# OPPO-Mente-Lab/X2I

Hardware: AMD Instinct MI355X
Metric: images/sec, FLUX-schnell 1024x1024 4-step (projector + denoise loop), whole job (higher is better)
Workload: dtype bf16; 1 GPU; BASELINE configs[1]: qwen3b conditioning (C=37,H=2048,S_txt=512) -> projector -> shuttle-3/FLUX-schnell DiT 1024x1024, 4 steps; batch_per_gpu=4, global_batch=4, parallelism=batch-sharded x1, graph=True

## Files before the change

x2i_amd/csrc/gemm256p.hip:

```cpp
#include <type_traits>
#include "gemm_device.h"
#include "gemm256p_epi.h"
#include "gemm256w_loop.inc"
#include "gemm256f8_loop.inc"

namespace x2i_gemm {
namespace {

__device__ __forceinline__ void epilogue_fx_slice(const GemmP& p, int z, int m_wave, int n_wave, int lane, char* stage, int slab0, int P, int j,
                                                  int tid) {
  typedef unsigned int u32x4 __attribute__((ext_vector_type(4)));
  typedef unsigned int u32x2 __attribute__((ext_vector_type(2)));
  const int mlane = lane & 15, ng = lane >> 4;
  const int srow = lane >> 3, sch = lane & 7;
  const float* b2 = p.bias2 ? p.bias2 + (long long)z * p.bias2_bs : nullptr;
#ifdef X2I_ABLATION
  if (p.act2 >= 80) b2 = nullptr;
#endif
  const float* gz = p.gate ? p.gate + (long long)z * p.gate_bs : nullptr;
  __amdgpu_buffer_rsrc_t r_rsrc = __builtin_amdgcn_make_buffer_rsrc((void*)(p.res + (long long)z * p.r_bs), 0, (uint32_t)(((long long)(p.M - 1) * p.ldr + p.N) * 2), 0x00020000);
  const uint32_t c_bytes = (uint32_t)(((long long)(p.M - 1) * p.ldc + p.N) * 2);
  __amdgpu_buffer_rsrc_t c_rsrc = __builtin_amdgcn_make_buffer_rsrc((void*)((bf16_t*)p.C + (long long)z * p.c_bs), 0, c_bytes, 0x00020000);
  const float* sbase = p.sk_slabs + (long long)slab0 * (SK_SLAB_BYTES / 4) + tid * 4;
  for (int q = j; q < 8; q += P) {
    const int h = q >> 2, c = q & 3;
    float bv[4][4], gv[4][4];
#pragma unroll
    for (int jj = 0; jj < 4; ++jj) {
      const int n = n_wave + h * 64 + jj * 16 + ng * 4;
#pragma unroll
      for (int r = 0; r < 4; ++r) bv[jj][r] = 0.f, gv[jj][r] = 1.f;
      if (n + 3 < p.N) {
        if (p.bias) {
          const uint2 bb = *(const uint2*)(p.bias + n);
          bv[jj][0] = __uint_as_float(bb.x << 16); bv[jj][1] = __uint_as_float(bb.x & 0xffff0000u);
          bv[jj][2] = __uint_as_float(bb.y << 16); bv[jj][3] = __uint_as_float(bb.y & 0xffff0000u);
        }
        if (gz) {
          const f32x4_t g4 = *(const f32x4_t*)(gz + n);
          gv[jj][0] = g4[0]; gv[jj][1] = g4[1]; gv[jj][2] = g4[2]; gv[jj][3] = g4[3];
        }
        if (b2) {
          const f32x4_t t4 = *(const f32x4_t*)(b2 + n);
          bv[jj][0] += t4[0]; bv[jj][1] += t4[1]; bv[jj][2] += t4[2]; bv[jj][3] += t4[3];
        }
      }
    }
    u32x2 rres[2][4];
    const uint32_t rsoff = (uint32_t)(((long long)c * 32 * p.ldr + h * 64) * 2);
#pragma unroll
    for (int i = 0; i < 2; ++i)
#pragma unroll
      for (int jj = 0; jj < 4; ++jj)
        rres[i][jj] = __builtin_amdgcn_raw_buffer_load_b64(r_rsrc, (uint32_t)(((long long)(m_wave + i * 16 + mlane) * p.ldr + n_wave + ng * 4) * 2) + jj * 32, rsoff, 0);
    f32x4_t sum[2][4];
    for (int u = 0; u < P; ++u) {
      const float* su = sbase + (long long)u * 8 * (SK_SLAB_BYTES / 4);
      f32x4_t v[2][4];
#pragma unroll
      for (int i = 0; i < 2; ++i)
#pragma unroll
        for (int jj = 0; jj < 4; ++jj) v[i][jj] = *(const f32x4_t*)(su + ((2 * c + i) * 8 + 4 * h + jj) * 1024);
#pragma unroll
      for (int i = 0; i < 2; ++i)
#pragma unroll
        for (int jj = 0; jj < 4; ++jj) sum[i][jj] = u ? sum[i][jj] + v[i][jj] : v[i][jj];
    }
#pragma unroll
    for (int i = 0; i < 2; ++i) {
      const int row = i * 16 + mlane;
#pragma unroll
      for (int jj = 0; jj < 4; ++jj) {
        float v[4];
#pragma unroll
        for (int r = 0; r < 4; ++r) v[r] = sum[i][jj][r] + bv[jj][r];
        const u32x2 r2 = rres[i][jj];
        v[0] = fmaf(gv[jj][0], v[0], __uint_as_float(r2[0] << 16));
        v[1] = fmaf(gv[jj][1], v[1], __uint_as_float(r2[0] & 0xffff0000u));
        v[2] = fmaf(gv[jj][2], v[2], __uint_as_float(r2[1] << 16));
        v[3] = fmaf(gv[jj][3], v[3], __uint_as_float(r2[1] & 0xffff0000u));
        char* slot = stage + row * 128 + ((((jj << 1) | (ng >> 1)) ^ ((row >> 1) & 7)) << 4) + ((ng & 1) << 3);
        *(uint2*)slot = make_uint2(pack_bf16x2(v[0], v[1]), pack_bf16x2(v[2], v[3]));
      }
    }
    asm volatile("s_waitcnt lgkmcnt(0)" ::: "memory");
    u32x4 d[4];
#pragma unroll
    for (int it = 0; it < 4; ++it) d[it] = *(const u32x4*)(stage + it * 1024 + lane * 16);
    const uint32_t soff = (uint32_t)((long long)c * 32 * p.ldc * 2);
#pragma unroll
    for (int it = 0; it < 4; ++it) {
      const int row = it * 8 + srow;
      const int n = n_wave + h * 64 + ((sch ^ ((row >> 1) & 7)) << 3);
      const uint32_t vo = (n + 7 < p.N) ? (uint32_t)(((long long)(m_wave + row) * p.ldc + n) * 2) : 0x80000000u;
      __builtin_amdgcn_raw_buffer_store_b128(d[it], c_rsrc, vo, soff, 0);
    }
    asm volatile("s_waitcnt lgkmcnt(0)" ::: "memory");
  }
}

template <bool F8 = false>
__device__ __forceinline__ void epilogue_qkv_chunked(const GemmP& p, f32x4_t (&acc)[2][4][2][4], int z, int m_wave, int n_wave, int lane,
                                                     char* stage, const Deq<F8>& dq) {
  asm volatile("" : "+v"(lane));
  const int mlane = lane & 15, ng = lane >> 4;
  const int Dm = p.q_H * 128;
  const int sec = n_wave / Dm;
  const int head = (n_wave - sec * Dm) >> 7;
  uint2 bvp[8];
  static_for<8>([&](auto jc) {
    constexpr int j = decltype(jc)::value;
    const int n = n_wave + j * 16 + ng * 4;
    bvp[j] = (p.bias && n + 3 < p.N) ? *(const uint2*)(p.bias + n) : make_uint2(0u, 0u);
  });
  auto bias_of = [&](int j, int r) {
    const uint32_t u = (r & 2) ? bvp[j].y : bvp[j].x;
    return __uint_as_float((r & 1) ? (u & 0xffff0000u) : (u << 16));
  };
  const TokMap tmap = tok_map(p, z, m_wave);
  auto token = [&](int m, int& b, int& st) { tok_of(tmap, m - m_wave, b, st); };
#ifdef X2I_QKV_ABL
  constexpr int qabl = X2I_QKV_ABL;
#else
  constexpr int qabl = 0;
#endif
  if constexpr (qabl == 92) {
    asm volatile("" ::X2I_GEMM256P_OPS_ACC_IN(acc));
    return;
  }
  if (sec < 2) {
    const int c = lane & 15, rsub = lane >> 4;
    float w[8];
    {
      const bf16x8_t wv = *(const bf16x8_t*)((sec ? p.q_nk : p.q_nq) + c * 8);
#pragma unroll
      for (int j = 0; j < 8; ++j) w[j] = bf16_to_f32((bf16_t)wv[j]) * (sec ? 1.f : p.q_qs);
    }
    typedef unsigned int u32x4 __attribute__((ext_vector_type(4)));
    __amdgpu_buffer_rsrc_t q_rsrc = __builtin_amdgcn_make_buffer_rsrc((void*)(sec ? p.q_K : p.q_Q), 0, 0x7ffffff0u, 0x00020000);
    __amdgpu_buffer_rsrc_t cos_rsrc = __builtin_amdgcn_make_buffer_rsrc((void*)p.q_cos, 0, 0x7ffffff0u, 0x00020000);
    __amdgpu_buffer_rsrc_t sin_rsrc = __builtin_amdgcn_make_buffer_rsrc((void*)p.q_sin, 0, 0x7ffffff0u, 0x00020000);
    auto qk_body = [&](auto pairs_c) {
    constexpr bool pairs = decltype(pairs_c)::value;
    f32x4_t cs[pairs ? 2 : 1][2][4];
    uint32_t qoff[pairs ? 2 : 1][2];
    auto load_cs = [&](int half, auto set_c) {
      constexpr int set = decltype(set_c)::value;
#pragma unroll
      for (int ps = 0; ps < 2; ++ps) {
        const int dm = half * 8 + ps * 4 + rsub;
        const bool valid = m_wave + dm < p.M;
        int b, st;
        tok_of(tmap, valid ? dm : 0, b, st);
        const uint32_t co = (uint32_t)(st * 128 + c * 8) * 4u;
        if constexpr (qabl == 86) {
          cs[set][ps][0] = cs[set][ps][1] = (f32x4_t){1.f, 1.f, 1.f, 1.f};
          cs[set][ps][2] = cs[set][ps][3] = (f32x4_t){0.f, 0.f, 0.f, 0.f};
        } else if constexpr (pairs) {
          cs[set][ps][0] = __builtin_bit_cast(f32x4_t, __builtin_amdgcn_raw_buffer_load_b128(cos_rsrc, co, 0, 0));
          cs[set][ps][1] = __builtin_bit_cast(f32x4_t, __builtin_amdgcn_raw_buffer_load_b128(cos_rsrc, co + 16, 0, 0));
        } else {
          cs[set][ps][0] = __builtin_bit_cast(f32x4_t, __builtin_amdgcn_raw_buffer_load_b128(cos_rsrc, co, 0, 0));
          cs[set][ps][1] = __builtin_bit_cast(f32x4_t, __builtin_amdgcn_raw_buffer_load_b128(cos_rsrc, co + 16, 0, 0));
          cs[set][ps][2] = __builtin_bit_cast(f32x4_t, __builtin_amdgcn_raw_buffer_load_b128(sin_rsrc, co, 0, 0));
          cs[set][ps][3] = __builtin_bit_cast(f32x4_t, __builtin_amdgcn_raw_buffer_load_b128(sin_rsrc, co + 16, 0, 0));
        }
        qoff[set][ps] = valid ? (uint32_t)(((b * p.q_H + head) * p.q_Spad + st) * 128 + c * 8) * 2u : 0x80000000u;
      }
    };
    auto park = [&](auto qc) {
      constexpr int q16 = decltype(qc)::value;
      constexpr int c2 = q16 >> 1, rr = q16 & 1;
      char* buf = stage + (q16 & 1) * 4096;
      static_for<2>([&](auto hc) {
        constexpr int h = decltype(hc)::value;
        static_for<4>([&](auto jc) {
          constexpr int j = decltype(jc)::value;
          float a[4];
#pragma unroll
          for (int r = 0; r < 4; ++r) {
            float t;
            asm volatile("v_accvgpr_read_b32 %0, %1" : "=v"(t) : "a"(acc[h][c2][rr][j][r]));
            if constexpr (F8) a[r] = fmaf(t * dq.sw[h * 4 + j][r], dq.sr[c2][rr], bias_of(h * 4 + j, r));
            else a[r] = t + bias_of(h * 4 + j, r);
          }
          *(uint2*)(buf + mlane * 256 + (((h * 8 + j * 2 + (ng >> 1)) ^ mlane) << 4) + ((ng & 1) << 3)) =
              make_uint2(pack_bf16x2(a[0], a[1]), pack_bf16x2(a[2], a[3]));
        });
      });
    };
    asm volatile("" ::: "memory");
    load_cs(0, std::integral_constant<int, 0>{});
    if constexpr (pairs) load_cs(1, std::integral_constant<int, 1>{});
    park(std::integral_constant<int, 0>{});
    static_for<8>([&](auto qc) {
      constexpr int q16 = decltype(qc)::value;
      char* buf = stage + (q16 & 1) * 4096;
      if constexpr (qabl == 90) {
        if constexpr (q16 + 1 < 8) park(std::integral_constant<int, q16 + 1>{});
        return;
      } else {
      __builtin_amdgcn_sched_barrier(0);
      asm volatile("s_waitcnt lgkmcnt(0)" ::: "memory");
      bf16x8_t xv[4];
#pragma unroll
      for (int k = 0; k < 4; ++k) {
        const int row = k * 4 + rsub;
        xv[k] = *(const bf16x8_t*)(buf + row * 256 + ((c ^ row) << 4));
      }
      __builtin_amdgcn_sched_barrier(0);
      static_for<2>([&](auto hfc) {
        constexpr int hf = decltype(hfc)::value;
        constexpr int half = 2 * q16 + hf;
        constexpr int set = pairs ? (half & 1) : 0;
        u32x4 outv[2];
        uint32_t so[2];
#pragma unroll
        for (int ps = 0; ps < 2; ++ps) {
          float x[8];
#pragma unroll
          for (int j = 0; j < 8; ++j) x[j] = bf16_to_f32((bf16_t)xv[hf * 2 + ps][j]);
          float ss = sumsq8(x);
          if constexpr (qabl != 87) {
#pragma unroll
          for (int o = 8; o > 0; o >>= 1) ss += __shfl_xor(ss, o, 64);
          }
          const float r = rms_rsqrt128(ss, p.q_eps);
          const f32x4_t t0 = cs[set][ps][0], t1 = cs[set][ps][1];
          float csv[8], snv[8];
          if constexpr (pairs) {
            csv[0] = csv[1] = t0[0]; snv[0] = snv[1] = t0[1]; csv[2] = csv[3] = t0[2]; snv[2] = snv[3] = t0[3];
            csv[4] = csv[5] = t1[0]; snv[4] = snv[5] = t1[1]; csv[6] = csv[7] = t1[2]; snv[6] = snv[7] = t1[3];
          } else {
            const f32x4_t t2 = cs[0][ps][2], t3 = cs[0][ps][3];
#pragma unroll
            for (int j = 0; j < 4; ++j) csv[j] = t0[j], csv[4 + j] = t1[j], snv[j] = t2[j], snv[4 + j] = t3[j];
          }
          float o8[8];
          norm_rope8(x, r, w, csv, snv, o8);
#pragma unroll
          for (int j = 0; j < 4; ++j) outv[ps][j] = pack_bf16x2(o8[2 * j], o8[2 * j + 1]);
          so[ps] = qoff[set][ps];
        }
        __builtin_amdgcn_sched_barrier(0);
        if constexpr (pairs) {
          if constexpr (half + 2 < 16) load_cs(half + 2, std::integral_constant<int, set>{});
        } else {
          if constexpr (half + 1 < 16) load_cs(half + 1, std::integral_constant<int, 0>{});
        }
        __builtin_amdgcn_sched_barrier(0);
        if constexpr (qabl != 88) {
#pragma unroll
        for (int ps = 0; ps < 2; ++ps) __builtin_amdgcn_raw_buffer_store_b128(outv[ps], q_rsrc, so[ps], 0, 0);
        } else {
          asm volatile("" ::"v"(outv[0]), "v"(outv[1]));
        }
      });
      if constexpr (q16 + 1 < 8) park(std::integral_constant<int, q16 + 1>{});
      }
    });
    };
    if (p.q_sin == nullptr) qk_body(std::true_type{});
    else qk_body(std::false_type{});
  } else {
    const int ch_lo = lane & 7, dp_lo = lane >> 3;
    const bool aligned = ((p.q_tok_off | p.q_rpb | p.q_row0 | p.M | p.q_Spad) & 7) == 0;
    auto fsw = [](int row) { return ((row >> 3) ^ (row >> 1)) & 7; };
    static_for<4>([&](auto qc) {
      constexpr int q = decltype(qc)::value;
      constexpr int h = q >> 1, cp = q & 1;
      __builtin_amdgcn_sched_barrier(0);
      static_for<2>([&](auto cc) {
        constexpr int c2 = 2 * cp + decltype(cc)::value;
        static_for<2>([&](auto rc) {
          constexpr int rr = decltype(rc)::value;
          const int row = decltype(cc)::value * 32 + rr * 16 + mlane;
          static_for<4>([&](auto jc) {
            constexpr int j = decltype(jc)::value;
            float a[4];
#pragma unroll
            for (int r = 0; r < 4; ++r) {
              float t;
              asm volatile("v_accvgpr_read_b32 %0, %1" : "=v"(t) : "a"(acc[h][c2][rr][j][r]));
              if constexpr (F8) a[r] = fmaf(t * dq.sw[h * 4 + j][r], dq.sr[c2][rr], bias_of(h * 4 + j, r));
              else a[r] = t + bias_of(h * 4 + j, r);
            }
            *(uint2*)(stage + row * 128 + (((j * 2 + (ng >> 1)) ^ fsw(row)) << 4) + ((ng & 1) << 3)) =
                make_uint2(pack_bf16x2(a[0], a[1]), pack_bf16x2(a[2], a[3]));
          });
        });
      });
      asm volatile("s_waitcnt lgkmcnt(0)" ::: "memory");
      if constexpr (qabl == 91) return;
#pragma unroll
      for (int it = 0; it < 4; ++it) {
        const int dp = it * 8 + dp_lo;
        uint32_t v[8];
#pragma unroll
        for (int k = 0; k < 8; ++k) {
          const int row = ch_lo * 8 + k;
          v[k] = *(const uint32_t*)(stage + row * 128 + (((dp >> 2) ^ fsw(row)) << 4) + ((dp & 3) << 2));
        }
        const int m = m_wave + cp * 64 + ch_lo * 8;
        if constexpr (qabl == 89) {
          asm volatile("" ::"v"(v[0]), "v"(v[1]), "v"(v[2]), "v"(v[3]), "v"(v[4]), "v"(v[5]), "v"(v[6]), "v"(v[7]));
        } else if (m < p.M) {
          const int d = h * 64 + dp * 2;
          int b, st;
          token(m, b, st);
          bf16_t* row0 = p.q_VT + (((long long)b * p.q_H + head) * 128 + d) * p.q_Spad;
          if (aligned) {
            union { bf16x8_t v8; uint32_t uu[4]; uint2 h2[2]; } lo, hi;
#pragma unroll
            for (int k = 0; k < 4; ++k) {
              lo.uu[k] = (v[2 * k] & 0xffffu) | (v[2 * k + 1] << 16);
              hi.uu[k] = (v[2 * k] >> 16) | (v[2 * k + 1] & 0xffff0000u);
            }
            if (p.q_vperm) {
              const int ps = x2i_vt_pos(st, 1);
              *(uint2*)(row0 + ps) = lo.h2[0]; *(uint2*)(row0 + ps + 8) = lo.h2[1];
              *(uint2*)(row0 + p.q_Spad + ps) = hi.h2[0]; *(uint2*)(row0 + p.q_Spad + ps + 8) = hi.h2[1];
            } else {
              *(bf16x8_t*)(row0 + st) = lo.v8;
              *(bf16x8_t*)(row0 + p.q_Spad + st) = hi.v8;
            }
          } else {
#pragma unroll
            for (int k = 0; k < 8; ++k) {
              if (m + k < p.M) {
                int bk, sk;
                token(m + k, bk, sk);
                bf16_t* rk = p.q_VT + (((long long)bk * p.q_H + head) * 128 + d) * p.q_Spad + x2i_vt_pos(sk, p.q_vperm);
                rk[0] = (bf16_t)(v[k] & 0xffffu);
                rk[p.q_Spad] = (bf16_t)(v[k] >> 16);
              }
            }
          }
        }
      }
      asm volatile("s_waitcnt lgkmcnt(0)" ::: "memory");
    });
  }
}

struct Unit {
  int vb, k0, len, slab;
  int kind = 0, tag = 0;
};

template <bool PAIR> using GemmArg = std::conditional_t<PAIR, GemmP2, GemmP>;
__device__ __forceinline__ const GemmP& prob(const GemmP& a, int) { return a; }
__device__ __forceinline__ const GemmP& first(const GemmP& a) { return a; }
__device__ __forceinline__ const GemmP& first(const GemmP2& a) { return a.p[0]; }
__device__ __forceinline__ const GemmP& second(const GemmP& a) { return a; }
__device__ __forceinline__ const GemmP& second(const GemmP2& a) { return a.p[1]; }
__device__ __forceinline__ GemmP prob(const GemmP2& a, int sel) {
  const GemmP &x = a.p[0], &y = a.p[1];
  GemmP q;
#define X2I_F(f) q.f = sel ? y.f : x.f;
  X2I_F(A) X2I_F(a_bs) X2I_F(lda) X2I_F(W) X2I_F(ldw) X2I_F(w_bs) X2I_F(bias) X2I_F(C) X2I_F(c_bs) X2I_F(ldc) X2I_F(C2) X2I_F(act2)
  X2I_F(gate) X2I_F(gate_bs) X2I_F(res) X2I_F(r_bs) X2I_F(ldr) X2I_F(bias2) X2I_F(bias2_bs) X2I_F(M) X2I_F(N) X2I_F(K) X2I_F(act)
  X2I_F(out_f32) X2I_F(tilesM) X2I_F(tilesN) X2I_F(cH) X2I_F(cW) X2I_F(cCin) X2I_F(cOW) X2I_F(cKW) X2I_F(cStride) X2I_F(cPad) X2I_F(cUp) X2I_F(cPadW) X2I_F(cRowPitch) X2I_F(cKorder) X2I_F(cMom) X2I_F(cMomBlocks)
  X2I_F(q_on) X2I_F(q_H) X2I_F(q_Spad) X2I_F(q_tok_off) X2I_F(q_rpb) X2I_F(q_row0) X2I_F(q_vperm) X2I_F(gm) X2I_F(q_eps) X2I_F(q_qs) X2I_F(q_nq) X2I_F(q_nk)
  X2I_F(q_cos) X2I_F(q_sin) X2I_F(q_Q) X2I_F(q_K) X2I_F(q_VT) X2I_F(f_sa) X2I_F(f_sa_bs) X2I_F(f_sw) X2I_F(f_alpha) X2I_F(f_oinv) X2I_F(f_out8)
  X2I_F(nbatch) X2I_F(sk_on) X2I_F(sk_slabs) X2I_F(sk_flags) X2I_F(fx_v0)
#undef X2I_F
  return q;
}

template <int ACT, bool RES, bool HASC2, bool QKV = false, bool PAIR = false, bool F8 = false, bool OUT8 = false, bool FX = false>
__global__ __launch_bounds__(256) void gemm256p_kernel(GemmArg<PAIR> pp) {
  constexpr int ES = F8 ? 1 : 2;
  constexpr int KT = F8 ? 128 : BK;
  extern __shared__ __attribute__((aligned(16))) char smem[];
  const GemmP& p = first(pp);
  const int tid = threadIdx.x;
  const int lane = tid & 63;
  const int wave = __builtin_amdgcn_readfirstlane(tid >> 6);
  const int wm = wave >> 1, wn = wave & 1;
  const int TT0 = p.tilesM * p.tilesN * p.nbatch;
  int TT = TT0;
  if constexpr (PAIR) TT += second(pp).tilesM * second(pp).tilesN * second(pp).nbatch;
  const int G = gridDim.x, w = blockIdx.x;
  const int nk = p.K / KT;

  auto tile_of = [&](int vb, int& sel, int& z, int& m0, int& n0) {
    sel = PAIR ? min(max(vb - TT0 + 1, 0), 1) : 0;
    const GemmP& q = prob(pp, sel);
    const int T = q.tilesM * q.tilesN;
    const int v = vb - sel * TT0;
    z = v / T;
    int bid = v - z * T;
    const int qq = T >> 3, r = T & 7, xcd = bid & 7, idx = bid >> 3;
    bid = (xcd < r ? xcd * (qq + 1) : r * (qq + 1) + (xcd - r) * qq) + idx;
    const int GM = q.gm;
    const int per_group = GM * q.tilesN;
    const int group = bid / per_group;
    const int first_m = group * GM;
    const int gsize = min(q.tilesM - first_m, GM);
    m0 = (first_m + (bid % per_group) % gsize) * BM2;
    n0 = ((bid % per_group) / gsize) * BN2;
  };
  const int khl = lane >> 5, r8 = (lane >> 2) & 7, cphys = lane & 3;
  const int kby = khl * 64 + ((cphys ^ (3 * (wave & 1))) << 4);
  auto offsets = [&](int sel, int z, int m0, int n0, uint32_t (&va)[8], uint32_t (&vw)[8]) {
    const GemmP& q = prob(pp, sel);
#ifdef X2I_ABLATION
    if (p.act2 == 75) m0 = 0, n0 = 0;
    if (p.act2 == 76) m0 &= 1023, n0 &= 2047;
#endif
    const long long zoff = (long long)z * q.a_bs;
#pragma unroll
    for (int jj = 0; jj < 8; ++jj) {
      const int row = (jj * 4 + wave) * 8 + r8;
      va[jj] = (m0 + row < q.M) ? (uint32_t)((zoff + (long long)(m0 + row) * q.lda) * ES + kby) : 0x80000000u;
      vw[jj] = (n0 + row < q.N) ? (uint32_t)(((long long)(n0 + row) * q.ldw) * ES + kby) : 0x80000000u;
    }
  };
  auto uni = [](auto v) { return (decltype(v))__builtin_amdgcn_readfirstlane((int)v); };
  auto mk_rsrc = [&](const void* ptr, uint32_t bytes) {
    const unsigned long long a = (unsigned long long)(uintptr_t)ptr;
    const unsigned long long au = ((unsigned long long)(unsigned)uni((int)(a >> 32)) << 32) | (unsigned)uni((int)(a & 0xffffffffu));
    return __builtin_amdgcn_make_buffer_rsrc((void*)(uintptr_t)au, 0, (uint32_t)uni((int)bytes), 0x00020000);
  };
  auto a_rsrc_of = [&](int sel) {
    const GemmP& q = prob(pp, sel);
    return mk_rsrc(q.A, (uint32_t)(((long long)(q.nbatch - 1) * q.a_bs + (long long)(q.M - 1) * q.lda + q.K) * ES));
  };
  auto w_rsrc_of = [&](int sel) {
    const GemmP& q = prob(pp, sel);
    return mk_rsrc(q.W, (uint32_t)(((long long)(q.N - 1) * q.ldw + q.K) * ES));
  };
  int fx_sel = 0, fx_Tp = 0, fx_nbz = 0, fx_kind = 0, fx_cnt = 0, fx_t0 = 0, fx_tstep = 1, fx_k0 = 0, fx_len = 0, fx_npre = 0, fx_modeB = 0, fx_slab_base = 0, fx_part = 0;
  const int fx_x = w & 7;
  if constexpr (FX) {
    const int wi = w >> 3, Gx = G >> 3;
    const int v0 = p.fx_v0;
    fx_sel = PAIR ? min(max(wi - v0 + 1, 0), 1) : 0;
    const GemmP& q = prob(pp, fx_sel);
    const int li = wi - fx_sel * v0, v = fx_sel ? Gx - v0 : v0;
    fx_Tp = q.tilesM * q.tilesN;
    fx_nbz = q.nbatch;
    fx_slab_base = fx_sel * (first(pp).tilesM * first(pp).tilesN);
    const int Tx = fx_Tp >> 3;
    if (v < 2 * Tx) {
      fx_modeB = 1;
      const int nt = v - Tx;
      const int tw = nt > 0 ? (Tx + nt - 1) / nt : 0;
      const int c = nt > 0 ? min(max(nk * tw / (tw + 1), 3), nk - 3) : nk;
      if (li < Tx) {
        fx_kind = 2; fx_cnt = 1; fx_t0 = li; fx_k0 = 0; fx_len = c; fx_npre = nt > 0 ? 1 : 0;
      } else {
        const int j = li - Tx;
        fx_kind = 1; fx_t0 = j; fx_tstep = nt; fx_cnt = (Tx - j + nt - 1) / nt; fx_k0 = c; fx_len = nk - c;
      }
    } else {
      const int base = v / Tx, extra = v - base * Tx;
      const int cutw = extra * (base + 1);
      const int t = li < cutw ? li / (base + 1) : extra + (li - cutw) / base;
      const int P = t < extra ? base + 1 : base;
      const int j = li < cutw ? li - t * (base + 1) : (li - cutw) - (t - extra) * base;
      const int k_lo = (int)((long long)nk * j / P), k_hi = (int)((long long)nk * (j + 1) / P);
      fx_cnt = 1; fx_t0 = t; fx_k0 = k_lo; fx_len = k_hi - k_lo;
      fx_kind = P > 1 ? 3 : 2;
      fx_npre = P - 1;
      fx_part = j;
    }
  }
  int S = TT / G;
  auto hasXlen = [](const Unit& u) { return u.len > 0; };
  Unit segH = {0, 0, 0, -1}, segX = {0, 0, 0, -1};
  int posX = 0;
  if (p.sk_on) {
    const int r = TT - S * G;
    const long long R = (long long)r * nk;
    const int Gp = (int)min((long long)G, R / 6);
    if (w < Gp) {
      auto snap = [&](long long b) {
        const int m = (int)(b % nk);
        return (m != 0 && m < 3) ? b - m : (m > nk - 3 ? b + (nk - m) : b);
      };
      const long long lo = snap(R * w / Gp), hi = snap(R * (w + 1) / Gp);
      if (hi > lo) {
        const int e0 = (int)(lo / nk), e1 = (int)((hi - 1) / nk);
        const int k0 = (int)(lo - (long long)e0 * nk);
        const Unit first = {S * G + e0, k0, (e1 > e0 ? nk : (int)(hi - (long long)e0 * nk)) - k0, e0};
        if (k0 == 0) segH = first; else segX = first;
        if (e1 > e0) segH = Unit{S * G + e1, 0, (int)(hi - (long long)e1 * nk), e1};
        if (segH.len == nk) segH.slab = -1;
        posX = hasXlen(segX) ? min(S, (int)((long long)S * segX.k0 / max(1, nk - segX.len))) : 0;
      }
    }
  } else if (w < TT - S * G) {
    S += 1;
  }
  const int hasH = segH.len > 0, hasX = segX.len > 0;
  const int n_units = FX ? fx_cnt * fx_nbz : S + hasH + hasX;
  auto unit = [&](int i) -> Unit {
    if constexpr (FX) {
      if (i >= n_units) return Unit{-1, 0, 0, -1};
      const int zi = i / fx_cnt, uu = i - zi * fx_cnt;
      const int tile = (fx_t0 + uu * fx_tstep) * 8 + fx_x;
      Unit u;
      u.vb = fx_sel * TT0 + zi * fx_Tp + tile;
      u.k0 = fx_k0;
      u.len = fx_len;
      u.slab = fx_modeB ? fx_slab_base + tile : (fx_kind == 1 ? w : (fx_kind == 3 ? w - 8 * fx_part : w - 8 * fx_npre));
      u.kind = fx_kind;
      u.tag = zi + 1;
      return Unit{uni(u.vb), uni(u.k0), uni(u.len), uni(u.slab), uni(u.kind), uni(u.tag)};
    }
    Unit u{w + (i - hasH) * G, 0, nk, -1};
    if (i >= n_units) u = Unit{-1, 0, 0, -1};
    else if (hasH && i == 0) u = segH;
    else if (hasX) {
      const int j = i - hasH;
      if (j == posX) u = segX;
      else if (j > posX) u.vb -= G;
    }
    return Unit{uni(u.vb), uni(u.k0), uni(u.len), uni(u.slab)};
  };


  const int frow = lane & 15;
  const uint32_t frag = (frow >> 3) * 1024 + (frow & 7) * 64 + (((lane >> 4) ^ (3 * ((frow >> 3) & 1))) << 4);
  uint32_t la = (uint32_t)(uintptr_t)smem + wm * 8 * 2048 + frag;
  uint32_t lw = (uint32_t)(uintptr_t)smem + 32768 + wn * 8 * 2048 + frag;
  uint32_t dma = __builtin_amdgcn_readfirstlane((uint32_t)(uintptr_t)smem + wave * 1024);
  char* stage = smem + P_STAGE_OFF + wave * P_STAGE_WAVE;
  const uint32_t slab_vo = (uint32_t)tid * 16;

  auto slab_rsrc = [&](int slab) {
    const unsigned long long a = (unsigned long long)(uintptr_t)p.sk_slabs + (unsigned long long)slab * SK_SLAB_BYTES;
    const unsigned long long au = ((unsigned long long)(unsigned)uni((int)(a >> 32)) << 32) | (unsigned)uni((int)(a & 0xffffffffu));
    return __builtin_amdgcn_make_buffer_rsrc((void*)(uintptr_t)au, 0, (uint32_t)SK_SLAB_BYTES, 0x00020000);
  };
  if (n_units == 0) return;
#ifdef X2I_ABLATION
  if (p.act2 >= 81 && p.act2 <= 85) {
    int n = (w & 7) * 10;
    if (p.act2 == 82) n = (((w * 167) & 255) * 80) >> 8;
    if (p.act2 == 83) n = (w & 7) * 5;
    if (p.act2 == 85) n = (w & 7) * 20;
    if (p.act2 == 84) {
      for (int i = 0; i < (w & 7) * 5; ++i) __builtin_amdgcn_s_sleep(13);
      n = 0;
    }
    for (int i = 0; i < n; ++i) __builtin_amdgcn_s_sleep(27);
  }
#endif
  auto fx_flag = [&](int buf, int slab) { return p.sk_flags + buf * 512 + slab; };
  auto fx_spin = [&](unsigned* f, unsigned want, unsigned shift, unsigned mask) {
    int spins = 0;
    while (((__hip_atomic_load(f, __ATOMIC_RELAXED, __HIP_MEMORY_SCOPE_AGENT) >> shift) & mask) != want) {
      __builtin_amdgcn_s_sleep(8);
      if (++spins > (1 << 22)) {
        __hip_atomic_store(p.sk_flags + SK_ERR_SLOT, 1u, __ATOMIC_RELAXED, __HIP_MEMORY_SCOPE_AGENT);
        break;
      }
    }
  };
  auto fx_reclaim = [&](int buf) {
    if (tid == 0) {
      fx_spin(fx_flag(buf, w), (unsigned)(fx_npre + 1), 0u, 0xffu);
      __hip_atomic_store(fx_flag(buf, w), 0u, __ATOMIC_RELAXED, __HIP_MEMORY_SCOPE_AGENT);
    }
    __syncthreads();
  };
  auto fx_slice_of = [&](int usel, int uz, int um0, int un0, int uslab0, int utag, int buf) {
    const int P = fx_npre + 1;
    if (tid == 0) {
      for (int q = 0; q < P; ++q) fx_spin(fx_flag(buf, uslab0 + 8 * q), (unsigned)utag, 8u, 0xffffffu);
      __builtin_amdgcn_fence(__ATOMIC_ACQUIRE, "agent");
    }
    __syncthreads();
    epilogue_fx_slice(prob(pp, usel), uz, um0 + wm * 128, un0 + wn * 128, lane, stage, uslab0 + 256 * buf, P, fx_part, tid);
    __syncthreads();
    if (tid == 0)
      for (int q = 0; q < P; ++q) __hip_atomic_fetch_add(fx_flag(buf, uslab0 + 8 * q), 1u, __ATOMIC_RELAXED, __HIP_MEMORY_SCOPE_AGENT);
  };
  int pend_valid = 0, pend_sel = 0, pend_z = 0, pend_m0 = 0, pend_n0 = 0, pend_slab0 = 0, pend_tag = 0;
  Unit cur = unit(0);
  int sel, z, m0, n0;
  tile_of(cur.vb, sel, z, m0, n0);
  uint32_t va[8], vw[8], na[8], nw[8];
  offsets(sel, z, m0, n0, va, vw);
  __amdgpu_buffer_rsrc_t a_rsrc = a_rsrc_of(sel), w_rsrc = w_rsrc_of(sel);
  bf16x8_t fr[F8 ? 1 : 32];
  uint32_t s_koff, s_it, s_so;
  int k0b = cur.k0 * 128;
  if constexpr (F8) {
    asm volatile(X2I_GEMM256F8_PRO
                 : [koff] "=&s"(s_koff)
                 : X2I_GEMM256W_OPS_VOFF(va, vw), [dma] "s"(dma), [ra] "s"(a_rsrc), [rw] "s"(w_rsrc), [k0b] "s"(k0b)
                 : "memory", "scc", "m0");
  } else {
    asm volatile(X2I_GEMM256P_PRO
                 : X2I_GEMM256P_OPS_FRAG0_OUT(fr), [koff] "=&s"(s_koff)
                 : X2I_GEMM256W_OPS_VOFF(va, vw), [la] "v"(la), [lw] "v"(lw), [dma] "s"(dma), [ra] "s"(a_rsrc), [rw] "s"(w_rsrc), [k0b] "s"(k0b)
                 : "memory", "scc", "m0");
  }
  for (int ui = 0;; ++ui) {
    const Unit nxt = unit(ui + 1);
    const bool has_next = nxt.vb >= 0;
    int nsel = PAIR ? min(max(nxt.vb - TT0 + 1, 0), 1) : 0, nz = 0, nm0 = 0, nn0 = 0;
    if constexpr (PAIR) a_rsrc = a_rsrc_of(sel), w_rsrc = w_rsrc_of(sel);
    const __amdgpu_buffer_rsrc_t na_rsrc = PAIR ? a_rsrc_of(nsel) : a_rsrc, nw_rsrc = PAIR ? w_rsrc_of(nsel) : w_rsrc;
    if (has_next) {
      tile_of(nxt.vb, nsel, nz, nm0, nn0);
      offsets(nsel, nz, nm0, nn0, na, nw);
    } else {
#pragma unroll
      for (int jj = 0; jj < 8; ++jj) na[jj] = nw[jj] = 0x80000000u;
    }
    const int nk0b = nxt.k0 * 128, len = cur.len;
    f32x4_t acc[2][4][2][4];
    const int fromp = FX ? 0 : min(cur.k0, 1);
    if (fromp) {
      unsigned* flag = p.sk_flags + cur.slab;
      if (tid == 0) {
        int spins = 0;
        while (__hip_atomic_load(flag, __ATOMIC_RELAXED, __HIP_MEMORY_SCOPE_AGENT) != (unsigned)cur.k0) {
          __builtin_amdgcn_s_sleep(32);
          if (++spins > (1 << 22)) {
            __hip_atomic_store(p.sk_flags + SK_ERR_SLOT, 1u, __ATOMIC_RELAXED, __HIP_MEMORY_SCOPE_AGENT);
            break;
          }
        }
        __builtin_amdgcn_fence(__ATOMIC_ACQUIRE, "agent");
      }
      __syncthreads();
    }
    __amdgpu_buffer_rsrc_t s_rsrc = slab_rsrc(cur.slab < 0 ? 0 : cur.slab);
    asm volatile(X2I_GEMM256P_LOAD_PARTIAL
                 : X2I_GEMM256P_OPS_ACC_OUT(acc), [so] "=&s"(s_so)
                 : [vo] "v"(slab_vo), [rs] "s"(s_rsrc), [fromp] "s"(fromp)
                 : "memory", "scc");
    const int zs = 1 - fromp;
    Deq<F8> dq;
    deq_load<F8>(prob(pp, sel), z, m0 + wm * 128, n0 + wn * 128, lane, dq);
#ifdef X2I_ABLATION
    unsigned long long* tdbg = (p.act2 >= 79 && tid == 0 && w < 16) ? (unsigned long long*)p.bias2 + w * 64 : nullptr;
    if (tdbg && ui < 31) tdbg[2 * ui] = __builtin_amdgcn_s_memrealtime();
#endif
    if constexpr (F8) {
      asm volatile(X2I_GEMM256F8_MAIN
                   : X2I_GEMM256P_OPS_ACC_IO(acc), [la] "+v"(la), [lw] "+v"(lw), [dma] "+s"(dma), [koff] "=&s"(s_koff), [it] "=&s"(s_it)
                   : X2I_GEMM256W_OPS_VOFF(va, vw), X2I_GEMM256P_OPS_NEXT(na, nw), [ra] "s"(a_rsrc), [rw] "s"(w_rsrc), [nra] "s"(na_rsrc),
                     [nrw] "s"(nw_rsrc), [nk] "s"(len), [k0b] "s"(k0b), [nk0b] "s"(nk0b), [zs] "s"(zs)
                   : "memory", "scc", "m0", X2I_GEMM256F8_FRAG_CLOBBERS);
    } else {
      asm volatile(X2I_GEMM256P_MAIN
                   : X2I_GEMM256P_OPS_ACC_IO(acc), X2I_GEMM256P_OPS_FRAG0_IO(fr), X2I_GEMM256P_OPS_FRAG1(fr), [la] "+v"(la), [lw] "+v"(lw),
                     [dma] "+s"(dma), [koff] "=&s"(s_koff), [it] "=&s"(s_it)
                   : X2I_GEMM256W_OPS_VOFF(va, vw), X2I_GEMM256P_OPS_NEXT(na, nw), [ra] "s"(a_rsrc), [rw] "s"(w_rsrc), [nra] "s"(na_rsrc),
                     [nrw] "s"(nw_rsrc), [nk] "s"(len),
                     [k0b] "s"(k0b), [nk0b] "s"(nk0b), [zs] "s"(zs)
                   : "memory", "scc", "m0");
    }
#ifdef X2I_ABLATION
    if (tdbg && ui < 31) tdbg[2 * ui + 1] = __builtin_amdgcn_s_memrealtime();
#endif
    auto spin_until = [&](unsigned* flag, unsigned want) {
      int spins = 0;
      while (__hip_atomic_load(flag, __ATOMIC_RELAXED, __HIP_MEMORY_SCOPE_AGENT) != want) {
        __builtin_amdgcn_s_sleep(32);
        if (++spins > (1 << 22)) {
          __hip_atomic_store(p.sk_flags + SK_ERR_SLOT, 1u, __ATOMIC_RELAXED, __HIP_MEMORY_SCOPE_AGENT);
          break;
        }
      }
    };
    if constexpr (FX) {
      if (cur.kind == 3) {
        const int buf = ui & 1;
        if (ui >= 2) fx_reclaim(buf);
        __amdgpu_buffer_rsrc_t s_rsrc = slab_rsrc(w + 256 * buf);
        asm volatile(X2I_GEMM256P_STORE_PARTIAL
                     : [so] "=&s"(s_so)
                     : X2I_GEMM256P_OPS_ACC_IN(acc), [vo] "v"(slab_vo), [rs] "s"(s_rsrc)
                     : "memory", "scc");
        __syncthreads();
        if (tid == 0) __hip_atomic_store(fx_flag(buf, w), (unsigned)cur.tag << 8, __ATOMIC_RELAXED, __HIP_MEMORY_SCOPE_AGENT);
        if (pend_valid) fx_slice_of(pend_sel, pend_z, pend_m0, pend_n0, pend_slab0, pend_tag, buf ^ 1);
        pend_valid = 1; pend_sel = sel; pend_z = z; pend_m0 = m0; pend_n0 = n0; pend_slab0 = cur.slab; pend_tag = cur.tag;
      } else if (cur.kind == 1) {
        if (tid == 0) spin_until(p.sk_flags + cur.slab, 0u);
        __syncthreads();
        __amdgpu_buffer_rsrc_t s_rsrc = slab_rsrc(cur.slab);
        asm volatile(X2I_GEMM256P_STORE_PARTIAL
                     : [so] "=&s"(s_so)
                     : X2I_GEMM256P_OPS_ACC_IN(acc), [vo] "v"(slab_vo), [rs] "s"(s_rsrc)
                     : "memory", "scc");
        __syncthreads();
        if (tid == 0) __hip_atomic_store(p.sk_flags + cur.slab, (unsigned)cur.tag, __ATOMIC_RELAXED, __HIP_MEMORY_SCOPE_AGENT);
      } else {
        const int npre = fx_npre;
        if (npre > 0) {
          if (tid == 0) {
            for (int q = 0; q < npre; ++q) spin_until(p.sk_flags + (cur.slab + 8 * q), (unsigned)cur.tag);
            __builtin_amdgcn_fence(__ATOMIC_ACQUIRE, "agent");
          }
          __syncthreads();
          epilogue_chunked_pipe<ACT, HASC2, RES, F8, true>(prob(pp, sel), acc, z, m0 + wm * 128, n0 + wn * 128, lane, stage, dq, cur.slab, npre, tid);
          __syncthreads();
          if (tid == 0)
            for (int q = 0; q < npre; ++q) __hip_atomic_store(p.sk_flags + (cur.slab + 8 * q), 0u, __ATOMIC_RELAXED, __HIP_MEMORY_SCOPE_AGENT);
        } else {
          epilogue_chunked_pipe<ACT, HASC2, RES, F8>(prob(pp, sel), acc, z, m0 + wm * 128, n0 + wn * 128, lane, stage, dq);
        }
      }
    } else if (cur.k0 + cur.len < nk) {
      __amdgpu_buffer_rsrc_t s_rsrc = slab_rsrc(cur.slab);
      asm volatile(X2I_GEMM256P_STORE_PARTIAL
                   : [so] "=&s"(s_so)
                   : X2I_GEMM256P_OPS_ACC_IN(acc), [vo] "v"(slab_vo), [rs] "s"(s_rsrc)
                   : "memory", "scc");
      __syncthreads();
      if (tid == 0) __hip_atomic_store(p.sk_flags + cur.slab, (unsigned)(cur.k0 + cur.len), __ATOMIC_RELAXED, __HIP_MEMORY_SCOPE_AGENT);
    } else {
      if (cur.k0 > 0 && tid == 0) __hip_atomic_store(p.sk_flags + cur.slab, 0u, __ATOMIC_RELAXED, __HIP_MEMORY_SCOPE_AGENT);
#ifdef X2I_ABLATION
      if (p.act2 == 77 || p.act2 == 79) {
        asm volatile("" ::X2I_GEMM256P_OPS_ACC_IN(acc));
      } else
#endif
      if constexpr (QKV) epilogue_qkv_chunked<F8>(prob(pp, sel), acc, z, m0 + wm * 128, n0 + wn * 128, lane, stage, dq);
      else if constexpr (OUT8) {
        if (p.f_oinv == 1.f) epilogue_chunked_pipe_e4m3<ACT, true>(prob(pp, sel), acc, z, m0 + wm * 128, n0 + wn * 128, lane, stage, dq);
        else epilogue_chunked_pipe_e4m3<ACT, false>(prob(pp, sel), acc, z, m0 + wm * 128, n0 + wn * 128, lane, stage, dq);
      } else epilogue_chunked_pipe<ACT, HASC2, RES, F8>(prob(pp, sel), acc, z, m0 + wm * 128, n0 + wn * 128, lane, stage, dq);
    }
    if (!has_next) break;
    cur = nxt; sel = nsel; z = nz; m0 = nm0; n0 = nn0; k0b = nk0b;

#pragma unroll
    for (int jj = 0; jj < 8; ++jj) va[jj] = na[jj], vw[jj] = nw[jj];
  }
  if constexpr (FX) {
    if (pend_valid) {
      const int last = (n_units - 1) & 1;
      fx_slice_of(pend_sel, pend_z, pend_m0, pend_n0, pend_slab0, pend_tag, last);
      if (n_units >= 2) fx_reclaim(last ^ 1);
      fx_reclaim(last);
    }
  }
  asm volatile(X2I_GEMM256P_DRAIN ::: "memory");
}

}

kern_t pick_gemm256p_qkv() { return gemm256p_kernel<X2I_ACT_NONE, false, false, true>; }

kern2_t pick_gemm256p_pair(int act, bool res, bool qkv, bool c2) {
  if (qkv) return gemm256p_kernel<X2I_ACT_NONE, false, false, true, true>;
  if (c2) return (act == X2I_ACT_NONE && !res) ? (kern2_t)gemm256p_kernel<X2I_ACT_NONE, false, true, false, true> : nullptr;
  if (res) return act == X2I_ACT_NONE ? (kern2_t)gemm256p_kernel<X2I_ACT_NONE, true, false, false, true> : nullptr;
  if (act == X2I_ACT_GELU_TANH) return gemm256p_kernel<X2I_ACT_GELU_TANH, false, false, false, true>;
  if (act == X2I_ACT_NONE) return gemm256p_kernel<X2I_ACT_NONE, false, false, false, true>;
  return nullptr;
}

kern_t pick_gemm256p_fp8(int act, bool res, bool out8, bool qkv) {
  if (qkv) return (!res && !out8 && act == X2I_ACT_NONE) ? (kern_t)gemm256p_kernel<X2I_ACT_NONE, false, false, true, false, true> : nullptr;
  if (out8) {
    if (res) return nullptr;
    if (act == X2I_ACT_NONE) return gemm256p_kernel<X2I_ACT_NONE, false, false, false, false, true, true>;
    if (act == X2I_ACT_GELU_TANH) return gemm256p_kernel<X2I_ACT_GELU_TANH, false, false, false, false, true, true>;
    return nullptr;
  }
  if (res) return act == X2I_ACT_NONE ? (kern_t)gemm256p_kernel<X2I_ACT_NONE, true, false, false, false, true> : nullptr;
  if (act == X2I_ACT_NONE) return gemm256p_kernel<X2I_ACT_NONE, false, false, false, false, true>;
  if (act == X2I_ACT_GELU_TANH) return gemm256p_kernel<X2I_ACT_GELU_TANH, false, false, false, false, true>;
  return nullptr;
}

kern_t pick_gemm256p_fx() { return gemm256p_kernel<X2I_ACT_NONE, true, false, false, false, false, false, true>; }
kern2_t pick_gemm256p_pair_fx() { return gemm256p_kernel<X2I_ACT_NONE, true, false, false, true, false, false, true>; }

kern_t pick_gemm256p(int act, bool res, bool f32, bool c2) {
  if (f32) return nullptr;
  if (res) return (act == X2I_ACT_NONE && !c2) ? (kern_t)gemm256p_kernel<X2I_ACT_NONE, true, false> : nullptr;
  if (c2) return act == X2I_ACT_NONE ? (kern_t)gemm256p_kernel<X2I_ACT_NONE, false, true> : nullptr;
  switch (act) {
    case X2I_ACT_NONE: return gemm256p_kernel<X2I_ACT_NONE, false, false>;
    case X2I_ACT_GELU_TANH: return gemm256p_kernel<X2I_ACT_GELU_TANH, false, false>;
    case X2I_ACT_GELU_ERF: return gemm256p_kernel<X2I_ACT_GELU_ERF, false, false>;
    case X2I_ACT_SILU: return gemm256p_kernel<X2I_ACT_SILU, false, false>;
    case X2I_ACT_RELU: return gemm256p_kernel<X2I_ACT_RELU, false, false>;
  }
  return nullptr;
}

}
```

Baseline: 4.574 images/s.

## Double-buffer V-transpose epilogue staging and use buffer stores for VT writes

Rewrites the V-section epilogue of the fused QKV GEMM so it runs in eight smaller chunks with two LDS stage buffers. Parking the next chunk's accumulators is interleaved with reading back and storing the current one. It uses a new swizzle function for the stage layout, computes token offsets once per four chunks, and writes the transposed V through raw buffer stores with a wave-uniform resource. With the permuted layout it can emit contiguous 16-byte runs. The aim is to hide LDS latency and cut per-store address arithmetic, at the cost of more complex indexing and an extra 4KB stage buffer.

```diff
diff --git a/x2i_amd/csrc/gemm256p.hip b/x2i_amd/csrc/gemm256p.hip
--- a/x2i_amd/csrc/gemm256p.hip
+++ b/x2i_amd/csrc/gemm256p.hip
@@ -97,6 +97,10 @@
     }
     asm volatile("s_waitcnt lgkmcnt(0)" ::: "memory");
   }
+}
+
+__host__ __device__ constexpr int vt_stage_off(int row, int dd) {
+  return ((((row & 0x38) | ((row ^ (row >> 2)) & 6) | ((row ^ (row >> 5)) & 1) | ((dd >> 2) << 6)) << 4) | (((dd & 3) ^ ((row >> 2) & 2)) << 2));
 }
 
 template <bool F8 = false>
@@ -263,20 +267,30 @@
     if (p.q_sin == nullptr) qk_body(std::true_type{});
     else qk_body(std::false_type{});
   } else {
-    const int ch_lo = lane & 7, dp_lo = lane >> 3;
-    const bool aligned = ((p.q_tok_off | p.q_rpb | p.q_row0 | p.M | p.q_Spad) & 7) == 0;
-    auto fsw = [](int row) { return ((row >> 3) ^ (row >> 1)) & 7; };
-    static_for<4>([&](auto qc) {
-      constexpr int q = decltype(qc)::value;
-      constexpr int h = q >> 1, cp = q & 1;
-      __builtin_amdgcn_sched_barrier(0);
+    typedef unsigned int u32x4 __attribute__((ext_vector_type(4)));
+    typedef unsigned int u32x2 __attribute__((ext_vector_type(2)));
+    const int geo = p.q_tok_off | p.q_rpb | p.q_row0 | p.M | p.q_Spad;
+    const bool al8 = (geo & 7) == 0;
+    const bool pmap = p.q_vperm && (geo & 31) == 0;
+    const bool run16 = pmap || (!p.q_vperm && al8);
+    const int g8 = lane & 7, dpl = lane >> 3;
+    const int trow = pmap ? 32 * (g8 >> 2) + 4 * (g8 & 3) : 8 * g8;
+    const int pbase = vt_stage_off(mlane, 2 * ng);
+    const int gbase = vt_stage_off(trow, dpl), gbase4 = gbase ^ vt_stage_off(pmap ? 16 : 4, 0);
+    const unsigned long long vta = (unsigned long long)(uintptr_t)(p.q_VT + ((long long)tmap.b0 * p.q_H + head) * 128 * p.q_Spad);
+    __amdgpu_buffer_rsrc_t vt_rsrc = __builtin_amdgcn_make_buffer_rsrc(
+        (void*)(uintptr_t)(((unsigned long long)(unsigned)__builtin_amdgcn_readfirstlane((int)(vta >> 32)) << 32) |
+                           (unsigned)__builtin_amdgcn_readfirstlane((int)(vta & 0xffffffffu))), 0, 0x7ffffff0u, 0x00020000);
+    uint32_t voff = 0x80000000u;
+    auto park = [&](auto nc) {
+      constexpr int n = decltype(nc)::value;
+      constexpr int cp = n >> 2, h = (n >> 1) & 1, jh = n & 1;
       static_for<2>([&](auto cc) {
-        constexpr int c2 = 2 * cp + decltype(cc)::value;
+        constexpr int cl = decltype(cc)::value, c2 = 2 * cp + cl;
         static_for<2>([&](auto rc) {
           constexpr int rr = decltype(rc)::value;
-          const int row = decltype(cc)::value * 32 + rr * 16 + mlane;
-          static_for<4>([&](auto jc) {
-            constexpr int j = decltype(jc)::value;
+          static_for<2>([&](auto jc) {
+            constexpr int jl = decltype(jc)::value, j = jh * 2 + jl;
             float a[4];
 #pragma unroll
             for (int r = 0; r < 4; ++r) {
@@ -285,60 +299,75 @@
               if constexpr (F8) a[r] = fmaf(t * dq.sw[h * 4 + j][r], dq.sr[c2][rr], bias_of(h * 4 + j, r));
               else a[r] = t + bias_of(h * 4 + j, r);
             }
-            *(uint2*)(stage + row * 128 + (((j * 2 + (ng >> 1)) ^ fsw(row)) << 4) + ((ng & 1) << 3)) =
+            *(uint2*)(stage + (n & 1) * 4096 + (pbase ^ vt_stage_off(cl * 32 + rr * 16, jl * 8))) =
                 make_uint2(pack_bf16x2(a[0], a[1]), pack_bf16x2(a[2], a[3]));
           });
         });
       });
+    };
+    asm volatile("" ::: "memory");
+    park(std::integral_constant<int, 0>{});
+    static_for<8>([&](auto nc) {
+      constexpr int n = decltype(nc)::value;
+      constexpr int cp = n >> 2, h = (n >> 1) & 1, jh = n & 1;
+      const char* buf = stage + (n & 1) * 4096;
+      __builtin_amdgcn_sched_barrier(0);
       asm volatile("s_waitcnt lgkmcnt(0)" ::: "memory");
-      if constexpr (qabl == 91) return;
-#pragma unroll
-      for (int it = 0; it < 4; ++it) {
-        const int dp = it * 8 + dp_lo;
-        uint32_t v[8];
-#pragma unroll
-        for (int k = 0; k < 8; ++k) {
-          const int row = ch_lo * 8 + k;
-          v[k] = *(const uint32_t*)(stage + row * 128 + (((dp >> 2) ^ fsw(row)) << 4) + ((dp & 3) << 2));
-        }
-        const int m = m_wave + cp * 64 + ch_lo * 8;
+      if constexpr (qabl == 91) {
+        if constexpr (n + 1 < 8) park(std::integral_constant<int, n + 1>{});
+        return;
+      } else {
+      uint32_t v[2][8];
+#pragma unroll
+      for (int it = 0; it < 2; ++it)
+#pragma unroll
+        for (int k = 0; k < 8; ++k) v[it][k] = *(const uint32_t*)(buf + ((k < 4 ? gbase : gbase4) ^ vt_stage_off(k & 3, 0)) + it * 2048);
+      __builtin_amdgcn_sched_barrier(0);
+      if constexpr (n + 1 < 8) park(std::integral_constant<int, n + 1>{});
+      __builtin_amdgcn_sched_barrier(0);
+      if constexpr ((n & 3) == 0) {
+        const int dm = cp * 64 + trow;
+        const bool valid = m_wave + dm < p.M;
+        int b, st;
+        tok_of(tmap, valid ? dm : 0, b, st);
+        voff = valid ? (uint32_t)((((b - tmap.b0) * p.q_H * 128 + 2 * dpl) * p.q_Spad + x2i_vt_pos(st, p.q_vperm)) * 2) : 0x80000000u;
+      }
+#pragma unroll
+      for (int it = 0; it < 2; ++it) {
         if constexpr (qabl == 89) {
-          asm volatile("" ::"v"(v[0]), "v"(v[1]), "v"(v[2]), "v"(v[3]), "v"(v[4]), "v"(v[5]), "v"(v[6]), "v"(v[7]));
-        } else if (m < p.M) {
-          const int d = h * 64 + dp * 2;
-          int b, st;
-          token(m, b, st);
-          bf16_t* row0 = p.q_VT + (((long long)b * p.q_H + head) * 128 + d) * p.q_Spad;
-          if (aligned) {
-            union { bf16x8_t v8; uint32_t uu[4]; uint2 h2[2]; } lo, hi;
-#pragma unroll
-            for (int k = 0; k < 4; ++k) {
-              lo.uu[k] = (v[2 * k] & 0xffffu) | (v[2 * k + 1] << 16);
-              hi.uu[k] = (v[2 * k] >> 16) | (v[2 * k + 1] & 0xffff0000u);
-            }
-            if (p.q_vperm) {
-              const int ps = x2i_vt_pos(st, 1);
-              *(uint2*)(row0 + ps) = lo.h2[0]; *(uint2*)(row0 + ps + 8) = lo.h2[1];
-              *(uint2*)(row0 + p.q_Spad + ps) = hi.h2[0]; *(uint2*)(row0 + p.q_Spad + ps + 8) = hi.h2[1];
-            } else {
-              *(bf16x8_t*)(row0 + st) = lo.v8;
-              *(bf16x8_t*)(row0 + p.q_Spad + st) = hi.v8;
-            }
+          asm volatile("" ::"v"(v[it][0]), "v"(v[it][1]), "v"(v[it][2]), "v"(v[it][3]), "v"(v[it][4]), "v"(v[it][5]), "v"(v[it][6]), "v"(v[it][7]));
+        } else if (al8) {
+          u32x4 lo, hi;
+#pragma unroll
+          for (int k = 0; k < 4; ++k) {
+            lo[k] = (v[it][2 * k] & 0xffffu) | (v[it][2 * k + 1] << 16);
+            hi[k] = (v[it][2 * k] >> 16) | (v[it][2 * k + 1] & 0xffff0000u);
+          }
+          const uint32_t so = (uint32_t)((h * 64 + jh * 32 + it * 16) * p.q_Spad * 2), so1 = so + (uint32_t)p.q_Spad * 2u;
+          if (run16) {
+            __builtin_amdgcn_raw_buffer_store_b128(lo, vt_rsrc, voff, so, 0);
+            __builtin_amdgcn_raw_buffer_store_b128(hi, vt_rsrc, voff, so1, 0);
           } else {
-#pragma unroll
-            for (int k = 0; k < 8; ++k) {
-              if (m + k < p.M) {
-                int bk, sk;
-                token(m + k, bk, sk);
-                bf16_t* rk = p.q_VT + (((long long)bk * p.q_H + head) * 128 + d) * p.q_Spad + x2i_vt_pos(sk, p.q_vperm);
-                rk[0] = (bf16_t)(v[k] & 0xffffu);
-                rk[p.q_Spad] = (bf16_t)(v[k] >> 16);
-              }
+            __builtin_amdgcn_raw_buffer_store_b64((u32x2){lo[0], lo[1]}, vt_rsrc, voff, so, 0);
+            __builtin_amdgcn_raw_buffer_store_b64((u32x2){lo[2], lo[3]}, vt_rsrc, voff + 16u, so, 0);
+            __builtin_amdgcn_raw_buffer_store_b64((u32x2){hi[0], hi[1]}, vt_rsrc, voff, so1, 0);
+            __builtin_amdgcn_raw_buffer_store_b64((u32x2){hi[2], hi[3]}, vt_rsrc, voff + 16u, so1, 0);
+          }
+        } else {
+          const int m = m_wave + cp * 64 + trow, d = h * 64 + jh * 32 + (it * 8 + dpl) * 2;
+#pragma unroll
+          for (int k = 0; k < 8; ++k) {
+            if (m + k < p.M) {
+              int bk, sk;
+              token(m + k, bk, sk);
+              bf16_t* rk = p.q_VT + (((long long)bk * p.q_H + head) * 128 + d) * p.q_Spad + x2i_vt_pos(sk, p.q_vperm);
+              rk[0] = (bf16_t)(v[it][k] & 0xffffu);
+              rk[p.q_Spad] = (bf16_t)(v[it][k] >> 16);
             }
           }
         }
       }
-      asm volatile("s_waitcnt lgkmcnt(0)" ::: "memory");
+      }
     });
   }
 }
```

Result: no change. 4.580 images/s (median of 6 runs) (+0.1%).
